# DinoBektesevic/lfd

Hardware: AMD Instinct MI355X
Metric: SDSS frames/sec (2048x1489) full detecttrails pipe (higher is better)
Workload: dtype f32

## Files before the change

lfd_amd/csrc/k_hough.h:

```cpp
#pragma once
#include "common.h"
#include "../../include/lfdmi.h"

#define PIXLIST_WORDS 8
#define CHUNK_MAX 64
__device__ __forceinline__ uint32_t chunk_entry(int y, int x0, int len) {
    return ((uint32_t)(len - 1) << 26) | ((uint32_t)y << 13) | (uint32_t)x0;
}

__global__ void __launch_bounds__(256)
k_pixlist(const u64 *bits0, const u64 *bits1, uint32_t *list0, uint32_t *list1, int *counters, int cm_a, int cm_b, int h, int w,
          size_t list_cap, int *accum_clear, int acc_n, size_t acc_stride, const int *active, int need_detect) {
    int g = blockIdx.y, im = blockIdx.z;
    const u64 *bits = im ? bits1 : bits0;
    uint32_t *list = im ? list1 : list0;
    const int cidx = im ? C_NPIX_BOX : C_NPIX_EQU, cidx_b = im ? C_NPIXB_BOX : C_NPIXB_EQU, nnz_idx = im ? C_NNZ_BOX : C_NNZ_EQU;
    if (accum_clear) accum_clear += (size_t)im * acc_stride;
    if (slot_off(active, counters, g)) return;
    int *cnt = counters + g * C_COUNT;
    if (need_detect && !cnt[C_DETECT]) return;
    int wq = LFD_WQ(w);
    if (accum_clear)
        for (int k = blockIdx.x * 256 + threadIdx.x; k < acc_n; k += gridDim.x * 256) accum_clear[(size_t)g * 2 * acc_stride + k] = 0;
    const int nw = h * wq;
// ... 199 lines not shown
    }
#undef LFD_BIN
    __syncthreads();
    int *ag = accum + ((size_t)g * 2 + im) * acc_cap;
    const int ts = numangle + 2;
    const int r0 = (numrho - 1) / 2 + lo;
    if (merge) {
        for (int k = threadIdx.x; k < nb * AW; k += NT) {
            int rr = r0 + (k >> aw_log2), al = k & (AW - 1);
            int v = acc[k];
            if (v && al < na) atomicAdd(&ag[(size_t)(rr + 1) * ts + a0 + al + 1], v);
        }
        return;
    }
    for (int k = threadIdx.x; k < (numrho + 2) * AW; k += NT) {
        int rr = (k >> aw_log2) - 1, al = k & (AW - 1);
        int rl = rr - r0;
        if (al < na) ag[(size_t)(rr + 1) * ts + a0 + al + 1] = (rl >= 0 && rl < nb) ? acc[rl * AW + al] : 0;
    }
    if (slab == 0)
        for (int k = threadIdx.x; k < numrho + 2; k += NT) { ag[(size_t)k * ts] = 0; ag[(size_t)k * ts + ts - 1] = 0; }
}

__global__ void __launch_bounds__(256)
k_hough_peaks(const int *accum, u64 *peaks, int *counters, int numangle, int numrho, int threshold,
              size_t acc_cap, size_t peak_cap, const int *active, int need_detect) {
    int g = blockIdx.z, im = blockIdx.y;
    if (slot_off(active, counters, g)) return;
    int *cnt = counters + g * C_COUNT;
    if (need_detect && !cnt[C_DETECT]) return;
    const int *ag = accum + ((size_t)g * 2 + im) * acc_cap;
    u64 *pg = peaks + ((size_t)g * 2 + im) * peak_cap;
    const int ts = numangle + 2;
    constexpr int PK_BUF = 4096;
    __shared__ u64 buf[PK_BUF];
    __shared__ int nbuf, gbase;
    if (threadIdx.x == 0) nbuf = 0;
    __syncthreads();
    auto flush = [&]() {
        const int nb = nbuf;
        if (threadIdx.x == 0 && nb) gbase = atomicAdd(&cnt[im ? C_NPEAK_BOX : C_NPEAK_EQU], nb);
        __syncthreads();
        for (int i = threadIdx.x; i < nb; i += (int)blockDim.x) {
            if ((size_t)(gbase + i) < peak_cap) pg[gbase + i] = buf[i];
            else cnt[C_OVERFLOW] = 1;
        }
        __syncthreads();
        if (threadIdx.x == 0) nbuf = 0;
        __syncthreads();
    };
    constexpr int RB = 8;
    const int per = ((numrho + (int)gridDim.x - 1) / (int)gridDim.x + RB - 1) / RB * RB;
    const int r0 = blockIdx.x * per, r1 = min(numrho, r0 + per);
    const int lane = threadIdx.x & 63, nth = (int)blockDim.x;
    int blk = 0;
    for (int n0 = 0; n0 < numangle; n0 += nth) {
        const int n = n0 + threadIdx.x;
        const bool on = n < numangle;
        const int *col = ag + (on ? n : 0) + 1;
        for (int rb = r0; rb < r1; rb += RB, blk++) {
            int v[RB + 2];
#pragma unroll
            for (int j = 0; j < RB + 2; j++) {
                const int rr = rb + j;
                v[j] = (on && rr <= numrho + 1) ? col[(size_t)rr * ts] : 0;
            }
#pragma unroll
            for (int j = 0; j < RB; j++) {
                const int r = rb + j, c = v[j + 1];
                int left = __shfl_up(c, 1), right = __shfl_down(c, 1);
                const bool cand = on && r < r1 && c > threshold && c > v[j] && c >= v[j + 2];
                if (cand) {
                    const int t = (r + 1) * ts + n + 1;
                    if (lane == 0) left = ag[t - 1];
                    if (lane == 63 || n == numangle - 1) right = ag[t + 1];
                    if (c > left && c >= right) {
                        const int base = (n + 1) * (numrho + 2) + r + 1;
                        buf[atomicAdd(&nbuf, 1)] = ((u64)(uint32_t)c << 32) | (u64)(uint32_t)(0x7fffffff - base);
                    }
                }
            }
            __syncthreads();
            if (nbuf > PK_BUF - RB * 256) flush();
            else __syncthreads();
        }
    }
    __syncthreads();
    flush();
}

__global__ void __launch_bounds__(256)
k_accum_untranspose(const int *accum, int *out, int numangle, int numrho, size_t acc_cap) {
    int g = blockIdx.y;
    const int *ag = accum + (size_t)g * 2 * acc_cap;
    int *og = out + (size_t)g * (numangle + 2) * (numrho + 2);
    int total = (numangle + 2) * (numrho + 2);
    for (int k = blockIdx.x * 256 + threadIdx.x; k < total; k += gridDim.x * 256) {
        int n1 = k / (numrho + 2), r1 = k - n1 * (numrho + 2);
        og[k] = ag[(size_t)r1 * (numangle + 2) + n1];
    }
}

__device__ __forceinline__ void key_to_line(u64 key, int numrho, float rho, float theta, float *orho,
                                            float *otheta) {
    int idx = 0x7fffffff - (int)(uint32_t)(key & 0xffffffffu);
    float scale = __fdiv_rn(1.f, (float)(numrho + 2));
    int n = (int)floorf(__fmul_rn((float)idx, scale)) - 1;
    int r = idx - (n + 1) * (numrho + 2) - 1;
    *orho = __fmul_rn(__fsub_rn((float)r, __fmul_rn((float)(numrho - 1), 0.5f)), rho);
    *otheta = __fadd_rn(0.f, __fmul_rn((float)n, theta));
}

__global__ void __launch_bounds__(256)
k_hough_topk(const u64 *peaks, const int *counters, float *lines, int K, int numrho, float rho,
             float theta, size_t peak_cap, const int *active, int need_detect) {
    int g = blockIdx.y, im = blockIdx.x;
    if (slot_off(active, counters, g)) return;
    const int *cnt = counters + g * C_COUNT;
    if (need_detect && !cnt[C_DETECT]) return;
    const u64 *pg = peaks + ((size_t)g * 2 + im) * peak_cap;
    int n = cnt[im ? C_NPEAK_BOX : C_NPEAK_EQU];
    if ((size_t)n > peak_cap) n = (int)peak_cap;
    __shared__ u64 red[4];
    __shared__ u64 prev_s;
    u64 prev = ~0ull;
    float *lg = lines + ((size_t)g * 2 + im) * K * 2;
    for (int round = 0; round < K; round++) {
        u64 best = 0;
        for (int k = threadIdx.x; k < n; k += 256) {
            u64 v = pg[k];
            if (v < prev && v > best) best = v;
        }
        for (int off = 32; off > 0; off >>= 1) {
            u64 o = __shfl_down(best, off);
            if (o > best) best = o;
        }
        if (lfd_lane() == 0) red[threadIdx.x >> 6] = best;
        __syncthreads();
        if (threadIdx.x == 0) {
            u64 b = red[0];
            for (int k = 1; k < 4; k++) if (red[k] > b) b = red[k];
            prev_s = b;
            float ro = 0.f, th = 0.f;
            if (b) key_to_line(b, numrho, rho, theta, &ro, &th);
            lg[2 * round] = ro;
            lg[2 * round + 1] = th;
        }
        __syncthreads();
        prev = prev_s;
        if (!prev) {
            if (threadIdx.x == 0)
                for (int r2 = round + 1; r2 < K; r2++) { lg[2 * r2] = 0.f; lg[2 * r2 + 1] = 0.f; }
            break;
        }
    }
}

__global__ void __launch_bounds__(1024)
k_hough_sort(u64 *peaks, const int *counters, float *lines, int max_lines, int numrho, float rho,
             float theta, size_t peak_cap) {
    int g = blockIdx.y, im = blockIdx.x;
    const int *cnt = counters + g * C_COUNT;
    if (cnt[C_OVERFLOW]) return;
    u64 *pg = peaks + ((size_t)g * 2 + im) * peak_cap;
    int n = cnt[im ? C_NPEAK_BOX : C_NPEAK_EQU];
    if ((size_t)n > peak_cap) n = (int)peak_cap;
    int np2 = 1;
    while (np2 < n) np2 <<= 1;
    for (int k = n + threadIdx.x; k < np2; k += 1024) pg[k] = 0;
    __syncthreads();
    for (int size = 2; size <= np2; size <<= 1)
        for (int stride = size >> 1; stride > 0; stride >>= 1) {
            for (int t = threadIdx.x; t < (np2 >> 1); t += 1024) {
                int lo = 2 * t - (t & (stride - 1));
                int hi = lo + stride;
                bool desc = ((lo & size) == 0);
                u64 a = pg[lo], b = pg[hi];
                if (desc ? (a < b) : (a > b)) { pg[lo] = b; pg[hi] = a; }
// ... 11 lines not shown
        for (int i = 0; i < n; i++) res = __dadd_rn(res, a[i]);
        return res;
    }
    double r[8], res;
    int i;
    for (int j = 0; j < 8; j++) r[j] = a[j];
    for (i = 8; i < n - (n % 8); i += 8)
        for (int j = 0; j < 8; j++) r[j] = __dadd_rn(r[j], a[i + j]);
    res = __dadd_rn(__dadd_rn(__dadd_rn(r[0], r[1]), __dadd_rn(r[2], r[3])),
                    __dadd_rn(__dadd_rn(r[4], r[5]), __dadd_rn(r[6], r[7])));
    for (; i < n; i++) res = __dadd_rn(res, a[i]);
    return res;
}
__device__ double np_mean_dev(const double *a, int n) {
    return __ddiv_rn(__dadd_rn(a[0], np_pairwise_dev(a + 1, n - 1)), (double)n);
}

struct TailParams {
    int navg;
    double dro, thetaTresh, lineSetTresh;
    int which;
};

__global__ void k_finalize(const float *lines, const int *counters, lfdmi_result *res, int *need_dim,
                           int *pass_flags, const int *active, TailParams tp, int G) {
    int g = blockIdx.x * blockDim.x + threadIdx.x;
    if (g >= G) return;
    if (active && !active[g]) { if (need_dim) need_dim[g] = 0; return; }
    const int *cnt = counters + g * C_COUNT;
    lfdmi_result r = res[g];
    r.detection = cnt[C_DETECT];
    r.rejected_by_theta = 0;
    r.n_lines_equ = r.n_lines_box = 0;
    if (cnt[C_OVERFLOW]) {
        r.status = LFDMI_ERR_CAPACITY;
        r.x1 = max(cnt[C_NRUNF], cnt[C_NRUNB]);
        r.y1 = cnt[C_NKEYS];
        r.x2 = cnt[C_NSLOTS];
        r.y2 = max(max(cnt[C_NPIX_EQU], cnt[C_NPIX_BOX]), max(cnt[C_NPIXB_EQU], cnt[C_NPIXB_BOX]));
        r.n_lines_equ = max(cnt[C_NPEAK_EQU], cnt[C_NPEAK_BOX]);
    }
    if (r.detection && r.status == 0) {
        int n1 = cnt[C_NPEAK_EQU], n2 = cnt[C_NPEAK_BOX];
        r.n_lines_equ = n1; r.n_lines_box = n2;
        if (n1 == 0 || n2 == 0) {
            r.status = LFDMI_ERR_NOLINES;
        } else {
            int K = tp.navg;
            const float *l1 = lines + ((size_t)g * 2 + 0) * K * 2, *l2 = lines + ((size_t)g * 2 + 1) * K * 2;
            double ro1[LFDMI_MAX_SET_LINES], ro2[LFDMI_MAX_SET_LINES], t1[LFDMI_MAX_SET_LINES],
                t2[LFDMI_MAX_SET_LINES];
            for (int i = 0; i < K; i++) {
                ro1[i] = ro2[i] = t1[i] = t2[i] = 0.;
                if (i >= n1) continue;
                ro1[i] = l1[2 * i];
                if (i >= n2) continue;
                ro2[i] = l2[2 * i];
                t1[i] = l1[2 * i + 1];
                t2[i] = l2[2 * i + 1];
            }
            bool rej = fabs(__dsub_rn(np_mean_dev(ro1, K), np_mean_dev(ro2, K))) > tp.dro;
            if (!rej) {
                double mx = t1[0], mn = t1[0];
                for (int i = 1; i < K; i++) { mx = fmax(mx, t1[i]); mn = fmin(mn, t1[i]); }
                rej = fabs(__dsub_rn(mx, mn)) > tp.thetaTresh;
            }
            if (!rej) {
                double mx = t2[0], mn = t2[0];
                for (int i = 1; i < K; i++) { mx = fmax(mx, t2[i]); mn = fmin(mn, t2[i]); }
                rej = fabs(__dsub_rn(mx, mn)) > tp.thetaTresh;
            }
            if (!rej) {
                for (int i = 0; i < K; i++) ro1[i] = fabs(__dsub_rn(t1[i], t2[i]));
                rej = np_mean_dev(ro1, K) > tp.lineSetTresh;
            }
            if (rej) r.rejected_by_theta = 1;
            else { r.found = tp.which; r.rho = l1[0]; r.theta = l1[1]; }
        }
    }
    res[g] = r;
    pass_flags[g] |= (tp.which == 1) ? (r.detection ? 1 : 0) : (2 | (r.detection ? 4 : 0));
    if (need_dim) need_dim[g] = (r.found == 0 && r.status == 0) ? 1 : 0;
}

__global__ void k_hough_reset(int *counters, int G) {
    int g = blockIdx.x * blockDim.x + threadIdx.x;
    if (g >= G) return;
    int *cnt = counters + g * C_COUNT;
    cnt[C_NPIX_EQU] = 0; cnt[C_NPIX_BOX] = 0; cnt[C_NPIXB_EQU] = 0; cnt[C_NPIXB_BOX] = 0; cnt[C_NPEAK_EQU] = 0; cnt[C_NPEAK_BOX] = 0;
    cnt[C_NNZ_EQU] = 0; cnt[C_NNZ_BOX] = 0;
}

__global__ void k_init_results(lfdmi_result *res, int *pass_flags, int G) {
    int g = blockIdx.x * blockDim.x + threadIdx.x;
    if (g >= G) return;
    pass_flags[g] = 0;
    lfdmi_result r;
    r.status = 0; r.found = 0; r.rho = 0.f; r.theta = 0.f;
    r.x1 = r.y1 = r.x2 = r.y2 = 0;
    r.n_lines_equ = r.n_lines_box = 0; r.detection = 0; r.rejected_by_theta = 0;
    res[g] = r;
}
```

lfd_amd/csrc/lfdmi.hip:

```cpp
#include <hip/hip_runtime.h>

#include <math.h>
#include <stdio.h>
#include <stdlib.h>
#include <time.h>
#include <pthread.h>
#include <sched.h>
#include <string.h>

#include <atomic>
#include <condition_variable>
#include <string>
#include <thread>
#include <mutex>
#include <memory>
#include <vector>

#include "../../include/lfdmi.h"
#include "common.h"
#include "k_ccl.h"
#include "k_hough.h"
#include "k_image.h"
#include "k_rect.h"
#include "k_frame.h"
#include "k_trail.h"
#include "fits_reader.h"
#include "unit.h"

#define LFD_PI 3.1415926535897932384626433832795
#define MAX_ANGLES 4096

enum {
    KID_REMOVESTARS = 0, KID_PREP_HIST, KID_LUT, KID_ERODE, KID_DILATE, KID_CANNY_NMS, KID_RUNS_INIT_FG,
    KID_RUNS_MERGE8, KID_RUNS_FLATTEN_FG, KID_EDGE, KID_RUNS_INIT_BG, KID_RUNS_MERGE4, KID_RUNS_FLATTEN_BG,
    KID_KEYS, KID_EXTREMES, KID_RECTS, KID_FILL, KID_PIXLIST, KID_VOTE, KID_PEAKS, KID_TOPK, KID_SORT,
    KID_FINALIZE, KID_DILATE_CANNY, KID_FRAME_FG, KID_FRAME_BG, KID_FRAME_KEYS, KID_PREP_ERODE, KID_PREP_DUAL, KID_BITS_ERODE, KID_MISC, TG_COUNT
};
static const char *const KID_NAMES[TG_COUNT] = {
    "k_removestars", "k_prep_hist", "k_lut", "k_morph(erode)", "k_morph(dilate)", "k_canny_nms", "k_runs_init(fg)",
    "k_runs_merge8", "k_runs_flatten(fg)", "k_edge_from_cand", "k_runs_init(bg)", "k_runs_merge4_bg",
    "k_runs_flatten(bg)", "k_keys", "k_extremes", "k_rects", "k_fill_quads", "k_pixlist", "k_hough_vote",
    "k_hough_peaks", "k_hough_topk", "k_hough_sort", "k_finalize", "k_dilate_canny", "k_frame_fg", "k_frame_bg",
    "k_frame_keys", "k_prep_erode", "k_prep_dual", "k_bits_erode", "misc"};

struct TimedSpan { hipEvent_t a, b; int group, pass, det; };

struct CallChunk {
    int c0, nc;
    bool general_on, scan_fused;
    long long growths;
};
struct PendingCall {
    int kind = 0;
// ... 70 lines not shown
    int *fb_fg = nullptr, *fb_bg = nullptr;
    int *perm = nullptr;
    const int *perm_cur = nullptr;
    bool use_perm = true;
    int *perm_tiles = nullptr;
    bool use_tile_perm = true;
    bool sky_fast = true;
    bool vote_classes = true;
    bool rs_fold_on = true;
    bool rs_fold = false;
    const int *rs_count_dev = nullptr; int rs_max_obj = 0;
    int rs_fill_at = 13;
    int rs_fill_at0 = 3, rs_fill_part = 0;
    float *rs_fill_frames = nullptr;
    int rs_fill_nc = 0, rs_fill_h = 0, rs_fill_w = 0;
    hipEvent_t ev_rsfill = nullptr;
    bool rs_fill_inflight = false;
    bool scan_fused = true;
    u64 *scan_partial = nullptr;
    int scan_epoch = 0;
    int scan_spin = 4096;
    bool rects_prep = true;
    bool vote_balance = true;
    lfdmi_result *res_dev = nullptr;
    void *res_host = nullptr;
    bool worst = false;
    lfdmi_ctx *spill = nullptr;
    long long n_spilled = 0;
    long long n_scan_giveups = 0, n_general_reruns = 0, n_general_chunks = 0, n_chunks = 0, n_cap_growths = 0;
    bool grow_on = true;
    bool scan_fused_cfg = true;
    int scan_quiet = 0, scan_rearm = 64;
    size_t bytes = 0;
    double min_rho = 1.0;
    void *scratch = nullptr;
    size_t scratch_bytes = 0;
    int last_h = 0, last_w = 0;
    int quiet_chunks = 0;
    void *feed_pin[2] = {nullptr, nullptr}, *feed_dev[2] = {nullptr, nullptr};
    size_t feed_bytes = 0, feed_pin_bytes = 0;
    bool feed_cpus_known = false;
    hipStream_t feed_copy = nullptr, feed_copy2 = nullptr;
    hipEvent_t feed_mid = nullptr;
    int feed_streams = 2;
    hipEvent_t feed_up[2] = {nullptr, nullptr};
    int feed_threads = 4;
// ... 245 lines not shown
    RET(dmalloc(ctx, &ctx->edgeb, G * BW));
    RET(dmalloc(ctx, &ctx->equb, G * BW));
    RET(dmalloc(ctx, &ctx->boxb, G * BW));
    RET(dmalloc(ctx, &ctx->dbits, G * BW));
    RET(dmalloc(ctx, &ctx->nzd, G * BW));
    for (int **p : {&ctx->Lf, &ctx->YMf, &ctx->FLf, &ctx->Lb, &ctx->YMb, &ctx->FLb, &ctx->SBf, &ctx->SBb, &ctx->PAb,
                    &ctx->ROWf, &ctx->ROWb})
        RET(dmalloc(ctx, p, G * ctx->run_cap));
    if (const char *e = getenv("LFDMI_DC_PROFILE")) ctx->dc_profile = atoi(e) != 0;
    if (const char *e = getenv("LFDMI_DC_SPECIALIZE")) ctx->dc_specialize = atoi(e) != 0;
    if (getenv("LFDMI_FRAME_PROFILE") || ctx->dc_profile) RET(dmalloc(ctx, &ctx->prof, G * 16));
    RET(dmalloc(ctx, &ctx->rsa, G * FRAME_RUNCAP));
    ctx->bm_bands = (max_h + CELLBM_ROWS - 1) / CELLBM_ROWS;
    if (const char *e = getenv("LFDMI_CELLBM")) ctx->use_cellbm = atoi(e) != 0;
    ctx->tile_cap = ((max_h + DCW_TH - 1) / DCW_TH) * ((max_w + CANNY_TW - 1) / CANNY_TW);
    RET(dmalloc(ctx, &ctx->tile_list, G * ctx->tile_cap));
    RET(dmalloc(ctx, &ctx->segcnt, G * SCAN_MAX_SEG));
    RET(dmalloc(ctx, &ctx->perm, G));
    RET(dmalloc(ctx, &ctx->perm_tiles, G));
    if (const char *e = getenv("LFDMI_TILE_PERM")) ctx->use_tile_perm = atoi(e) != 0;
    if (const char *e = getenv("LFDMI_SKY_FAST")) ctx->sky_fast = atoi(e) != 0;
    if (const char *e = getenv("LFDMI_VOTE_CLASSES")) ctx->vote_classes = atoi(e) != 0;
    if (const char *e = getenv("LFDMI_VOTE_BALANCE")) ctx->vote_balance = atoi(e) != 0;
    if (const char *e = getenv("LFDMI_RECTS_PREP")) ctx->rects_prep = atoi(e) != 0;
    if (const char *e = getenv("LFDMI_RS_FOLD")) ctx->rs_fold_on = atoi(e) != 0;
    if (const char *e = getenv("LFDMI_RS_SORT_MIN")) ctx->rs_sort_min = atoi(e);
    if (const char *e = getenv("LFDMI_SCAN_FUSED")) ctx->scan_fused = atoi(e) != 0;
    ctx->scan_fused_cfg = ctx->scan_fused;
    if (const char *e = getenv("LFDMI_GROW")) ctx->grow_on = atoi(e) != 0;
    if (const char *e = getenv("LFDMI_SCAN_REARM")) ctx->scan_rearm = std::max(1, atoi(e));
    if (const char *e = getenv("LFDMI_SCAN_SPIN")) ctx->scan_spin = std::max(0, atoi(e));
    if (const char *e = getenv("LFDMI_SCAN_EPOCH0")) ctx->scan_epoch = atoi(e) & ((1 << 22) - 1);
    if (const char *e = getenv("LFDMI_RS_FILL_AT")) ctx->rs_fill_at = atoi(e);
    if (const char *e = getenv("LFDMI_RS_FILL_AT0")) ctx->rs_fill_at0 = atoi(e);
    if (const char *e = getenv("LFDMI_PERM")) ctx->use_perm = atoi(e) != 0;
    RET(dmalloc(ctx, &ctx->fb_fg, G));
    RET(dmalloc(ctx, &ctx->fg_keys, G));
    HIPCHK(hipMemsetAsync(ctx->fg_keys, 0, G * sizeof(int), ctx->stream));
    if (const char *e = getenv("LFDMI_FG_KEYS")) ctx->fg_keys_on = atoi(e) != 0;
    RET(dmalloc(ctx, &ctx->fb_bg, G));
    RET(dmalloc(ctx, &ctx->scanf_, G * BW));
    RET(dmalloc(ctx, &ctx->scanb_, G * BW));
    RET(dmalloc(ctx, &ctx->keys, G * ctx->key_cap));
    RET(dmalloc(ctx, &ctx->bigkeys, G * ctx->key_cap));
    RET(dmalloc(ctx, &ctx->medkeys, G * ctx->key_cap));
    RET(dmalloc(ctx, &ctx->wl_fg, G * BW));
// ... 15 lines not shown
        ctx->counters = (int *)(blk + nb_bm + nb_hist);
        ctx->zero_block = blk;
        ctx->zero_bytes = nb_bm + nb_hist + nb_cnt;
        ctx->zero_counters_off = nb_bm + nb_hist;
        uint8_t *blk2 = nullptr;
        RET(dmalloc(ctx, &blk2, nb_bm + nb_hist));
        ctx->cellbm2 = (u64 *)blk2;
        ctx->hist2 = (int *)(blk2 + nb_bm);
        ctx->zero_block2 = blk2;
        ctx->zero_bytes2 = nb_bm + nb_hist;
        RET(dmalloc(ctx, &ctx->fullbits, G * (size_t)max_h * ((max_w + 255) >> 8)));
        RET(dmalloc(ctx, &ctx->candmask, G * (size_t)((max_h + MORPH_TH - 1) / MORPH_TH) * 2));
    }
    RET(dmalloc(ctx, &ctx->need_dim, G));
    RET(dmalloc(ctx, &ctx->scan_partial, G * SCAN_MAX_BLK));
    HIPCHK(hipMemsetAsync(ctx->scan_partial, 0, G * SCAN_MAX_BLK * sizeof(u64), ctx->stream));
    {
        char *blk = nullptr;
        RET(dmalloc(ctx, &blk, G * sizeof(int) + G * LFDMI_MAX_SCALES * sizeof(lfdmi_result)));
        ctx->pass_flags = (int *)blk;
        ctx->res_dev = (lfdmi_result *)(blk + G * sizeof(int));
        HIPCHK(hipHostMalloc(&ctx->res_host, G * sizeof(int) + G * sizeof(lfdmi_result), hipHostMallocDefault));
    }
    HIPCHK(hipFuncSetAttribute((const void *)k_hough_vote<6>, hipFuncAttributeMaxDynamicSharedMemorySize, 160 * 1024 - 64));
    HIPCHK(hipFuncSetAttribute((const void *)k_hough_vote<5>, hipFuncAttributeMaxDynamicSharedMemorySize, 160 * 1024 - 64));
    HIPCHK(hipFuncSetAttribute((const void *)k_hough_vote<4>, hipFuncAttributeMaxDynamicSharedMemorySize, 160 * 1024 - 64));
    HIPCHK(hipFuncSetAttribute((const void *)k_hough_vote<3>, hipFuncAttributeMaxDynamicSharedMemorySize, 160 * 1024 - 64));
    HIPCHK(hipFuncSetAttribute((const void *)k_hough_vote<2>, hipFuncAttributeMaxDynamicSharedMemorySize, 160 * 1024 - 64));
    HIPCHK(hipFuncSetAttribute((const void *)k_hough_vote<1>, hipFuncAttributeMaxDynamicSharedMemorySize, 160 * 1024 - 64));
    HIPCHK(hipFuncSetAttribute((const void *)k_hough_vote<0>, hipFuncAttributeMaxDynamicSharedMemorySize, 160 * 1024 - 64));
    HIPCHK(hipFuncSetAttribute((const void *)k_rects_big, hipFuncAttributeMaxDynamicSharedMemorySize, 160 * 1024 - 64));
    HIPCHK(hipFuncSetAttribute((const void *)k_dilate_canny_v, hipFuncAttributeMaxDynamicSharedMemorySize, 64 * 1024));
    HIPCHK(hipFuncSetAttribute((const void *)k_frame_fg, hipFuncAttributeMaxDynamicSharedMemorySize, 160 * 1024 - 1024));
    HIPCHK(hipFuncSetAttribute((const void *)k_prep_erode<false, 0>, hipFuncAttributeMaxDynamicSharedMemorySize, 140 * 1024));
    HIPCHK(hipFuncSetAttribute((const void *)k_prep_erode<false, 1>, hipFuncAttributeMaxDynamicSharedMemorySize, 140 * 1024));
    HIPCHK(hipFuncSetAttribute((const void *)k_prep_erode<false, 2>, hipFuncAttributeMaxDynamicSharedMemorySize, 140 * 1024));
    HIPCHK(hipFuncSetAttribute((const void *)k_prep_erode<false, 3>, hipFuncAttributeMaxDynamicSharedMemorySize, 140 * 1024));
    HIPCHK(hipFuncSetAttribute((const void *)k_prep_erode<true, LFDMI_PREP_BRIGHT_THEN_DIM>, hipFuncAttributeMaxDynamicSharedMemorySize, 140 * 1024));
    HIPCHK(hipFuncSetAttribute((const void *)k_frame_contours, hipFuncAttributeMaxDynamicSharedMemorySize,
                               (FRAME_RUNCAP + 4 * (FRAME_RUNCAP / 32)) * (int)sizeof(int)));
    HIPCHK(hipFuncSetAttribute((const void *)k_morph_rect<0>, hipFuncAttributeMaxDynamicSharedMemorySize, 64 * 1024));
    HIPCHK(hipFuncSetAttribute((const void *)k_morph_rect<1>, hipFuncAttributeMaxDynamicSharedMemorySize, 64 * 1024));
    return 0;
}

extern "C" int lfdmi_ctx_create(int device, int max_h, int max_w, int max_inflight, lfdmi_ctx **out) {
// ... 729 lines not shown
    float rho = (float)rho_d, theta = (float)theta_d;
    if (!(rho > 0) || !(theta > 0)) return fail(ctx, LFDMI_ERR_ARG, "rho and theta must be positive");
    int na, nr;
    lfdmi_hough_dims(h, w, rho_d, theta_d, &na, &nr);
    if (na <= 0 || nr <= 0 || na > MAX_ANGLES || (size_t)(na + 2) * (nr + 2) > ctx->acc_cap)
        return fail(ctx, LFDMI_ERR_CAPACITY, "Hough accumulator larger than the workspace (rho < 1 px or theta < 1 deg)");
    int slot = 0;
    for (int i = 1; i < LFDMI_MAX_SCALES; i++) if (ctx->tabs[i].stamp < ctx->tabs[slot].stamp) slot = i;
    auto &t = ctx->tabs[slot];
    t.host.assign((size_t)2 * na, 0.f);
    float irho = 1 / rho;
    float ang = 0.f;
    for (int n = 0; n < na; ang += theta, n++) {
        t.host[n] = (float)(cos((double)ang) * irho);
        t.host[na + n] = (float)(sin((double)ang) * irho);
    }
    HIPCHK(hipMemcpyAsync(ctx->tab + (size_t)slot * 2 * MAX_ANGLES, t.host.data(), t.host.size() * sizeof(float), hipMemcpyHostToDevice, ctx->stream));
    t.rho = rho_d; t.theta = theta_d; t.h = h; t.w = w; t.numangle = na; t.numrho = nr;
    t.stamp = ++ctx->tab_clock;
    ctx->tab_cur = slot; ctx->numangle = na; ctx->numrho = nr;
    return 0;
}

static int run_hough(lfdmi_ctx *ctx, int nc, int h, int w, double rho, double theta, int threshold, int n_img, int K,
                     int need_detect, const int *active) {
    RET(ensure_tables(ctx, h, w, rho, theta));
    int na = ctx->numangle, nr = ctx->numrho;
    const std::vector<float> &tab_host = ctx->tabs[ctx->tab_cur].host;
    const int half = (nr - 1) / 2;
    VoteRanges rng;
    int aw_log2 = 6, nslabs = 1, nbmax = nr;
    const bool have_tab = (int)tab_host.size() == 2 * na;
    auto slab_ranges = [&](int awl) {
        int AW = 1 << awl;
        nslabs = (na + AW - 1) / AW;
        nbmax = 1;
        for (int sl = 0; sl < VOTE_MAX_SLABS; sl++) { rng.lo[sl] = -half - 1; rng.hi[sl] = nr - half; }
        if (nslabs <= VOTE_MAX_SLABS && have_tab) {
            for (int sl = 0; sl < nslabs; sl++) {
                double rmin = 0, rmax = 0;
                for (int n = sl * AW; n < na && n < (sl + 1) * AW; n++) {
                    double c = tab_host[n], sn = tab_host[na + n];
                    for (int cx = 0; cx < 2; cx++)
                        for (int cy = 0; cy < 2; cy++) {
                            double r = (cx ? w : 0) * c + (cy ? h : 0) * sn;
                            rmin = r < rmin ? r : rmin;
                            rmax = r > rmax ? r : rmax;
                        }
// ... 61 lines not shown
                                                                    h, w, ctx->list_cap, (nsplit > 1 || balance) ? ctx->accum : nullptr, acc_n, ctx->acc_cap,
                                                                    active, need_detect);
        KCHK("k_pixlist"); }
        Span sp(ctx, KID_VOTE, need_detect);
        const int vsplit = balance ? 2 * nsplit : nsplit;
        dim3 vgrid(nslabs * vsplit, balance ? 1 : n_img, nc);
        size_t vlds = ((size_t)nbmax << aw_log2) * 4 + 256;
        static const int vote_threads_env = getenv("LFDMI_VOTE_THREADS") ? std::max(64, std::min(1024, atoi(getenv("LFDMI_VOTE_THREADS")) & ~63)) : 0;
        const int vote_threads = vote_threads_env ? vote_threads_env : (narrow_path ? VOTE_THREADS / 2 : VOTE_THREADS);
#define LFD_LAUNCH_VOTE(L)                                                                                          \
    case L:                                                                                                         \
        k_hough_vote<L><<<vgrid, vote_threads, vlds, ctx->stream>>>(ctx->pix_equ, ctx->pix_box, ctx->counters,           \
                                                                   ctx->tab + (size_t)ctx->tab_cur * 2 * MAX_ANGLES, \
                                                                   ctx->accum, na, nr, vsplit, ctx->list_cap,       \
                                                                   ctx->acc_cap, active, need_detect, rng, balance); \
        break;
        switch (aw_log2) {
            LFD_LAUNCH_VOTE(6) LFD_LAUNCH_VOTE(5) LFD_LAUNCH_VOTE(4) LFD_LAUNCH_VOTE(3) LFD_LAUNCH_VOTE(2)
            LFD_LAUNCH_VOTE(1) LFD_LAUNCH_VOTE(0)
        }
#undef LFD_LAUNCH_VOTE
        KCHK("k_hough_vote");
    }
    { Span sp(ctx, KID_PEAKS, need_detect);
    static const int peak_rows = getenv("LFDMI_PEAK_ROWS") ? std::max(8, atoi(getenv("LFDMI_PEAK_ROWS"))) : 32;
    k_hough_peaks<<<dim3(std::min(32, std::max(1, nr / peak_rows)), n_img, nc), std::min(256, (na + 63) / 64 * 64), 0, ctx->stream>>>(ctx->accum, ctx->peaks, ctx->counters, na, nr, threshold,
                                                                ctx->acc_cap, ctx->peak_cap, active, need_detect);
    KCHK("k_hough_peaks"); }
    if (K > 0) {
        Span sp(ctx, KID_TOPK, need_detect);
        k_hough_topk<<<dim3(n_img, nc), 256, 0, ctx->stream>>>(ctx->peaks, ctx->counters, ctx->lines, K, nr, (float)rho, (float)theta,
                                                               ctx->peak_cap, active, need_detect);
        KCHK("k_hough_topk");
    }
    return 0;
}

static int check_params(lfdmi_ctx *ctx, const lfdmi_params *p, bool dim) {
    if (!p) return fail(ctx, LFDMI_ERR_ARG, "params NULL");
    if (p->gaussKernel < 0 || p->gaussKernel > 31 || (p->gaussKernel > 0 && (p->gaussKernel & 1) == 0))
        return fail(ctx, LFDMI_ERR_ARG, "gaussKernel must be 0 (off) or odd, 1..31");
    if (p->nlinesInSet < 1 || p->nlinesInSet > LFDMI_MAX_SET_LINES) return fail(ctx, LFDMI_ERR_ARG, "nlinesInSet out of range");
    if (!p->dilateKernel) return fail(ctx, LFDMI_ERR_ARG, "dilateKernel NULL");
    if (dim && !p->erodeKernel) return fail(ctx, LFDMI_ERR_ARG, "erodeKernel NULL");
    return 0;
}

static int prep_erode_rows(const lfdmi_ctx *ctx, int w, int kh) {
    int BR = ctx->pe_rows;
// ... 117 lines not shown
    }
    if (p->gaussKernel > 0) {
        RET(run_morph(ctx, dil_src, ctx->equ, ctx->equb, ctx->lut, p->dilateKernel, p->dilate_kh, p->dilate_kw, 0, nc, h, w, active));
        RET(ensure_scratch(ctx, (size_t)ctx->G * ctx->N));
        RET(run_gauss(ctx, ctx->equ, (uint8_t *)ctx->scratch, nc, h, w, p->gaussKernel, p->gaussSigma, active));
        RET(run_canny(ctx, (const uint8_t *)ctx->scratch, nc, h, w, 0, 255, active, false, true));
    } else if (can_fuse_dilate_canny(p->dilateKernel, p->dilate_kh, p->dilate_kw, w)) {
        RET(run_dilate_canny(ctx, dil_src, nc, h, w, ctx->lut, p->dilate_kh, p->dilate_kw, active, ctx->use_cellbm ? bm : nullptr));
        RET(rs_fill_point(ctx, 2 + 10 * ctx->cur_pass));
        RET(run_canny(ctx, ctx->equ, nc, h, w, 0, 255, active, true, true));
    } else {
        RET(run_morph(ctx, dil_src, ctx->equ, ctx->equb, ctx->lut, p->dilateKernel, p->dilate_kh, p->dilate_kw, 0, nc, h, w, active));
        RET(run_canny(ctx, ctx->equ, nc, h, w, 0, 255, active, false, true));
    }
    return run_rects(ctx, nc, h, w, p->contoursMode, p->contoursMethod, p->minAreaRectMinLen, p->lwTresh, active);
}

static int run_tail(lfdmi_ctx *ctx, int nc, int h, int w, double rho, bool dim, const lfdmi_params *p, const int *active,
                    int *need_dim, lfdmi_result *res, bool again) {
    if (again) {
        k_hough_reset<<<(nc + 63) / 64, 64, 0, ctx->stream>>>(ctx->counters, nc);
        KCHK("k_hough_reset");
    }
    RET(run_hough(ctx, nc, h, w, rho, LFD_PI / 180, 1, 2, p->nlinesInSet, 1, active));
    TailParams tp;
    tp.navg = p->nlinesInSet; tp.dro = p->dro; tp.thetaTresh = p->thetaTresh; tp.lineSetTresh = p->lineSetTresh;
    tp.which = dim ? 2 : 1;
    Span sp(ctx, KID_FINALIZE);
    k_finalize<<<(nc + 63) / 64, 64, 0, ctx->stream>>>(ctx->lines, ctx->counters, res, need_dim, ctx->pass_flags, active, tp, nc);
    KCHK("k_finalize");
    return 0;
}

static int run_pass(lfdmi_ctx *ctx, const void *src, int dtype, int nc, int h, int w, int flip, int prep_mode, bool dim,
                    const lfdmi_params *p, const int *active, int *need_dim, const lfdmi_params *dual_dim = nullptr) {
    RET(run_front(ctx, src, dtype, nc, h, w, flip, prep_mode, dim, p, active, dual_dim));
    ctx->perm_cur = nullptr;
    return run_tail(ctx, nc, h, w, p->houghMethod, dim, p, active, need_dim, ctx->res_dev, false);
}

static void dictify(int h, int w, lfdmi_result *r) {
    if (!r->found) return;
    float c = cosf(r->theta), s = sinf(r->theta);
    float x0 = c * r->rho, y0 = s * r->rho;
    float L = (float)(h + w);
    r->x1 = (int32_t)(x0 - L * s);
    r->y1 = (int32_t)(y0 + L * c);
    r->x2 = (int32_t)(x0 + L * s);
    r->y2 = (int32_t)(y0 - L * c);
}
// ... 1271 lines not shown
    HIPCHK(hipSetDevice(ctx->device));
    const int G = ctx->G, K = navg;
    std::vector<float> lines((size_t)G * 2 * K * 2);
    std::vector<int> cnt((size_t)G * C_COUNT);
    for (int c0 = 0; c0 < n; c0 += G) {
        const int nc = std::min(G, n - c0);
        std::fill(lines.begin(), lines.end(), 0.f);
        std::fill(cnt.begin(), cnt.end(), 0);
        for (int i = 0; i < nc; i++) {
            const int a = n1[c0 + i], b = n2[c0 + i];
            if (a < 0 || a > kmax || b < 0 || b > kmax) return fail(ctx, LFDMI_ERR_ARG, "lfdmi_debug_tail: line count");
            for (int k = 0; k < K && k < a; k++) { lines[((size_t)i * 2 + 0) * K * 2 + 2 * k] = h1[((size_t)(c0 + i) * kmax + k) * 2]; lines[((size_t)i * 2 + 0) * K * 2 + 2 * k + 1] = h1[((size_t)(c0 + i) * kmax + k) * 2 + 1]; }
            for (int k = 0; k < K && k < b; k++) { lines[((size_t)i * 2 + 1) * K * 2 + 2 * k] = h2[((size_t)(c0 + i) * kmax + k) * 2]; lines[((size_t)i * 2 + 1) * K * 2 + 2 * k + 1] = h2[((size_t)(c0 + i) * kmax + k) * 2 + 1]; }
            cnt[(size_t)i * C_COUNT + C_DETECT] = 1;
            cnt[(size_t)i * C_COUNT + C_NPEAK_EQU] = a;
            cnt[(size_t)i * C_COUNT + C_NPEAK_BOX] = b;
        }
        HIPCHK(hipMemcpyAsync(ctx->lines, lines.data(), (size_t)nc * 2 * K * 2 * sizeof(float), hipMemcpyHostToDevice, ctx->stream));
        HIPCHK(hipMemcpyAsync(ctx->counters, cnt.data(), (size_t)nc * C_COUNT * sizeof(int), hipMemcpyHostToDevice, ctx->stream));
        k_init_results<<<(nc + 63) / 64, 64, 0, ctx->stream>>>(ctx->res_dev, ctx->pass_flags, nc);
        KCHK("k_init_results");
        TailParams tp;
        tp.navg = navg; tp.dro = dro; tp.thetaTresh = thetaTresh; tp.lineSetTresh = lineSetTresh; tp.which = which;
        k_finalize<<<(nc + 63) / 64, 64, 0, ctx->stream>>>(ctx->lines, ctx->counters, ctx->res_dev, nullptr, ctx->pass_flags, nullptr, tp, nc);
        KCHK("k_finalize");
        HIPCHK(hipMemcpyAsync(out + c0, ctx->res_dev, (size_t)nc * sizeof(lfdmi_result), hipMemcpyDeviceToHost, ctx->stream));
        HIPCHK(hipStreamSynchronize(ctx->stream));
        for (int i = 0; i < nc; i++) dictify(h, w, &out[c0 + i]);
    }
    return 0;
}

extern "C" int lfdmi_debug_trig(lfdmi_ctx *ctx, int n, const double *y, const double *x, float *angle_deg, float *cos_half, float *sin_half) {
    if (!ctx || n < 0 || !y || !x || !angle_deg || !cos_half || !sin_half) return LFDMI_ERR_ARG;
    RET(idle(ctx));
    if (n == 0) return 0;
    HIPCHK(hipSetDevice(ctx->device));
    RET(ensure_scratch(ctx, (size_t)n * (2 * sizeof(double) + 3 * sizeof(float))));
    double *dy = (double *)ctx->scratch, *dx = dy + n;
    float *o = (float *)(dx + n);
    HIPCHK(hipMemcpyAsync(dy, y, (size_t)n * sizeof(double), hipMemcpyHostToDevice, ctx->stream));
    HIPCHK(hipMemcpyAsync(dx, x, (size_t)n * sizeof(double), hipMemcpyHostToDevice, ctx->stream));
    k_debug_trig<<<(n + 255) / 256, 256, 0, ctx->stream>>>(dy, dx, o, o + n, o + 2 * (size_t)n, n);
    KCHK("k_debug_trig");
    HIPCHK(hipMemcpyAsync(angle_deg, o, (size_t)n * sizeof(float), hipMemcpyDeviceToHost, ctx->stream));
    HIPCHK(hipMemcpyAsync(cos_half, o + n, (size_t)n * sizeof(float), hipMemcpyDeviceToHost, ctx->stream));
    HIPCHK(hipMemcpyAsync(sin_half, o + 2 * (size_t)n, (size_t)n * sizeof(float), hipMemcpyDeviceToHost, ctx->stream));
    HIPCHK(hipStreamSynchronize(ctx->stream));
// ... 213 lines not shown
```

Baseline: 62780.

## Vectorize Hough peak scan and add optional fused peaks/topk/finalize tail kernel

```diff
diff --git a/lfd_amd/csrc/k_hough.h b/lfd_amd/csrc/k_hough.h
--- a/lfd_amd/csrc/k_hough.h
+++ b/lfd_amd/csrc/k_hough.h
@@ -245,6 +245,74 @@
         for (int k = threadIdx.x; k < numrho + 2; k += NT) { ag[(size_t)k * ts] = 0; ag[(size_t)k * ts + ts - 1] = 0; }
 }
 
+#define PEAK_ST 4
+__device__ __forceinline__ unsigned peak_item(const int *ag, int ts, int numangle, int r, int n0, int threshold, int *votes) {
+    const int *row = ag + (size_t)(r + 1) * ts + n0 + 1;
+    int c[PEAK_ST + 2], lo[PEAK_ST], hi[PEAK_ST];
+    if (n0 + PEAK_ST <= numangle) {
+        __builtin_memcpy(&c[1], row, PEAK_ST * sizeof(int));
+        __builtin_memcpy(lo, row - ts, PEAK_ST * sizeof(int));
+        __builtin_memcpy(hi, row + ts, PEAK_ST * sizeof(int));
+        c[0] = row[-1];
+        c[PEAK_ST + 1] = row[PEAK_ST];
+    } else {
+        c[0] = row[-1];
+#pragma unroll
+        for (int j = 0; j <= PEAK_ST; j++) c[j + 1] = (n0 + j <= numangle) ? row[j] : 0;
+#pragma unroll
+        for (int j = 0; j < PEAK_ST; j++) {
+            lo[j] = (n0 + j < numangle) ? row[j - ts] : 0;
+            hi[j] = (n0 + j < numangle) ? row[j + ts] : 0;
+        }
+    }
+    unsigned m = 0;
+#pragma unroll
+    for (int j = 0; j < PEAK_ST; j++) {
+        const int v = c[j + 1];
+        votes[j] = v;
+        if (n0 + j < numangle && v > threshold && v > lo[j] && v >= hi[j] && v > c[j] && v >= c[j + 2]) m |= 1u << j;
+    }
+    return m;
+}
+
+__device__ __forceinline__ void peaks_append(u64 *list, size_t cap, int *n, unsigned mask, const int *votes, int r, int n0, int numrho) {
+    const int lane = lfd_lane();
+    int off[PEAK_ST], total = 0;
+#pragma unroll
+    for (int j = 0; j < PEAK_ST; j++) {
+        const u64 bal = __ballot((mask >> j) & 1u);
+        off[j] = total + __popcll(bal & ((1ull << lane) - 1ull));
+        total += __popcll(bal);
+    }
+    if (total == 0) return;
+    int base = 0;
+    if (lane == 0) base = atomicAdd(n, total);
+    base = __shfl(base, 0);
+#pragma unroll
+    for (int j = 0; j < PEAK_ST; j++)
+        if ((mask >> j) & 1u) {
+            const int pos = base + off[j], cell = (n0 + j + 1) * (numrho + 2) + r + 1;
+            if ((size_t)pos < cap) list[pos] = ((u64)(uint32_t)votes[j] << 32) | (u64)(uint32_t)(0x7fffffff - cell);
+        }
+}
+
+__device__ __forceinline__ void peaks_scan(const int *ag, int numangle, int numrho, int threshold, int i_beg, int i_end, u64 *list,
+                                           size_t cap, int *n) {
+    const int ts = numangle + 2, nq = (numangle + PEAK_ST - 1) / PEAK_ST, nth = (int)blockDim.x;
+    for (int i0 = i_beg; i0 < i_end; i0 += nth) {
+        const int it = i0 + (int)threadIdx.x;
+        int votes[PEAK_ST] = {0, 0, 0, 0}, r = 0, n0 = 0;
+        unsigned m = 0;
+        if (it < i_end) {
+            const int dr = it / nq;
+            r = dr;
+            n0 = (it - dr * nq) * PEAK_ST;
+            m = peak_item(ag, ts, numangle, r, n0, threshold, votes);
+        }
+        peaks_append(list, cap, n, m, votes, r, n0, numrho);
+    }
+}
+
 __global__ void __launch_bounds__(256)
 k_hough_peaks(const int *accum, u64 *peaks, int *counters, int numangle, int numrho, int threshold,
               size_t acc_cap, size_t peak_cap, const int *active, int need_detect) {
@@ -254,8 +322,7 @@
     if (need_detect && !cnt[C_DETECT]) return;
     const int *ag = accum + ((size_t)g * 2 + im) * acc_cap;
     u64 *pg = peaks + ((size_t)g * 2 + im) * peak_cap;
-    const int ts = numangle + 2;
-    constexpr int PK_BUF = 4096;
+    constexpr int PK_BUF = 4096, PK_ROUND = 256 * PEAK_ST;
     __shared__ u64 buf[PK_BUF];
     __shared__ int nbuf, gbase;
     if (threadIdx.x == 0) nbuf = 0;
@@ -272,41 +339,14 @@
         if (threadIdx.x == 0) nbuf = 0;
         __syncthreads();
     };
-    constexpr int RB = 8;
-    const int per = ((numrho + (int)gridDim.x - 1) / (int)gridDim.x + RB - 1) / RB * RB;
-    const int r0 = blockIdx.x * per, r1 = min(numrho, r0 + per);
-    const int lane = threadIdx.x & 63, nth = (int)blockDim.x;
-    int blk = 0;
-    for (int n0 = 0; n0 < numangle; n0 += nth) {
-        const int n = n0 + threadIdx.x;
-        const bool on = n < numangle;
-        const int *col = ag + (on ? n : 0) + 1;
-        for (int rb = r0; rb < r1; rb += RB, blk++) {
-            int v[RB + 2];
-#pragma unroll
-            for (int j = 0; j < RB + 2; j++) {
-                const int rr = rb + j;
-                v[j] = (on && rr <= numrho + 1) ? col[(size_t)rr * ts] : 0;
-            }
-#pragma unroll
-            for (int j = 0; j < RB; j++) {
-                const int r = rb + j, c = v[j + 1];
-                int left = __shfl_up(c, 1), right = __shfl_down(c, 1);
-                const bool cand = on && r < r1 && c > threshold && c > v[j] && c >= v[j + 2];
-                if (cand) {
-                    const int t = (r + 1) * ts + n + 1;
-                    if (lane == 0) left = ag[t - 1];
-                    if (lane == 63 || n == numangle - 1) right = ag[t + 1];
-                    if (c > left && c >= right) {
-                        const int base = (n + 1) * (numrho + 2) + r + 1;
-                        buf[atomicAdd(&nbuf, 1)] = ((u64)(uint32_t)c << 32) | (u64)(uint32_t)(0x7fffffff - base);
-                    }
-                }
-            }
-            __syncthreads();
-            if (nbuf > PK_BUF - RB * 256) flush();
-            else __syncthreads();
-        }
+    const int per = (numrho + (int)gridDim.x - 1) / (int)gridDim.x;
+    const int r0 = min(numrho, (int)blockIdx.x * per), r1 = min(numrho, r0 + per);
+    const int nq = (numangle + PEAK_ST - 1) / PEAK_ST, i1 = r1 * nq;
+    for (int i0 = r0 * nq; i0 < i1; i0 += 256) {
+        peaks_scan(ag, numangle, numrho, threshold, i0, min(i1, i0 + 256), buf, PK_BUF, &nbuf);
+        __syncthreads();
+        if (nbuf > PK_BUF - PK_ROUND) flush();
+        else __syncthreads();
     }
     __syncthreads();
     flush();
@@ -332,6 +372,43 @@
     int r = idx - (n + 1) * (numrho + 2) - 1;
     *orho = __fmul_rn(__fsub_rn((float)r, __fmul_rn((float)(numrho - 1), 0.5f)), rho);
     *otheta = __fadd_rn(0.f, __fmul_rn((float)n, theta));
+}
+
+#define TOPK_MAX_WAVES 16
+__device__ __forceinline__ void topk_rounds(const u64 *pg, int n, float *lg, int K, int numrho, float rho, float theta,
+                                            u64 *red, u64 *prev_s_) {
+    u64 &prev_s = *prev_s_;
+    const int nth = (int)blockDim.x, nwv = nth >> 6;
+    u64 prev = ~0ull;
+    for (int round = 0; round < K; round++) {
+        u64 best = 0;
+        for (int k = threadIdx.x; k < n; k += nth) {
+            u64 v = pg[k];
+            if (v < prev && v > best) best = v;
+        }
+        for (int off = 32; off > 0; off >>= 1) {
+            u64 o = __shfl_down(best, off);
+            if (o > best) best = o;
+        }
+        if (lfd_lane() == 0) red[threadIdx.x >> 6] = best;
+        __syncthreads();
+        if (threadIdx.x == 0) {
+            u64 b = red[0];
+            for (int k = 1; k < nwv; k++) if (red[k] > b) b = red[k];
+            prev_s = b;
+            float ro = 0.f, th = 0.f;
+            if (b) key_to_line(b, numrho, rho, theta, &ro, &th);
+            lg[2 * round] = ro;
+            lg[2 * round + 1] = th;
+        }
+        __syncthreads();
+        prev = prev_s;
+        if (!prev) {
+            if (threadIdx.x == 0)
+                for (int r2 = round + 1; r2 < K; r2++) { lg[2 * r2] = 0.f; lg[2 * r2 + 1] = 0.f; }
+            break;
+        }
+    }
 }
 
 __global__ void __launch_bounds__(256)
@@ -344,39 +421,9 @@
     const u64 *pg = peaks + ((size_t)g * 2 + im) * peak_cap;
     int n = cnt[im ? C_NPEAK_BOX : C_NPEAK_EQU];
     if ((size_t)n > peak_cap) n = (int)peak_cap;
-    __shared__ u64 red[4];
+    __shared__ u64 red[TOPK_MAX_WAVES];
     __shared__ u64 prev_s;
-    u64 prev = ~0ull;
-    float *lg = lines + ((size_t)g * 2 + im) * K * 2;
-    for (int round = 0; round < K; round++) {
-        u64 best = 0;
-        for (int k = threadIdx.x; k < n; k += 256) {
-            u64 v = pg[k];
-            if (v < prev && v > best) best = v;
-        }
-        for (int off = 32; off > 0; off >>= 1) {
-            u64 o = __shfl_down(best, off);
-            if (o > best) best = o;
-        }
-        if (lfd_lane() == 0) red[threadIdx.x >> 6] = best;
-        __syncthreads();
-        if (threadIdx.x == 0) {
-            u64 b = red[0];
-            for (int k = 1; k < 4; k++) if (red[k] > b) b = red[k];
-            prev_s = b;
-            float ro = 0.f, th = 0.f;
-            if (b) key_to_line(b, numrho, rho, theta, &ro, &th);
-            lg[2 * round] = ro;
-            lg[2 * round + 1] = th;
-        }
-        __syncthreads();
-        prev = prev_s;
-        if (!prev) {
-            if (threadIdx.x == 0)
-                for (int r2 = round + 1; r2 < K; r2++) { lg[2 * r2] = 0.f; lg[2 * r2 + 1] = 0.f; }
-            break;
-        }
-    }
+    topk_rounds(pg, n, lines + ((size_t)g * 2 + im) * K * 2, K, numrho, rho, theta, red, &prev_s);
 }
 
 __global__ void __launch_bounds__(1024)
@@ -434,10 +481,8 @@
     int which;
 };
 
-__global__ void k_finalize(const float *lines, const int *counters, lfdmi_result *res, int *need_dim,
-                           int *pass_flags, const int *active, TailParams tp, int G) {
-    int g = blockIdx.x * blockDim.x + threadIdx.x;
-    if (g >= G) return;
+__device__ __forceinline__ void finalize_slot(int g, const float *lines, const int *counters, lfdmi_result *res, int *need_dim,
+                                              int *pass_flags, const int *active, const TailParams &tp, double *work) {
     if (active && !active[g]) { if (need_dim) need_dim[g] = 0; return; }
     const int *cnt = counters + g * C_COUNT;
     lfdmi_result r = res[g];
@@ -460,8 +505,7 @@
         } else {
             int K = tp.navg;
             const float *l1 = lines + ((size_t)g * 2 + 0) * K * 2, *l2 = lines + ((size_t)g * 2 + 1) * K * 2;
-            double ro1[LFDMI_MAX_SET_LINES], ro2[LFDMI_MAX_SET_LINES], t1[LFDMI_MAX_SET_LINES],
-                t2[LFDMI_MAX_SET_LINES];
+            double *ro1 = work, *ro2 = work + LFDMI_MAX_SET_LINES, *t1 = work + 2 * LFDMI_MAX_SET_LINES, *t2 = work + 3 * LFDMI_MAX_SET_LINES;
             for (int i = 0; i < K; i++) {
                 ro1[i] = ro2[i] = t1[i] = t2[i] = 0.;
                 if (i >= n1) continue;
@@ -493,6 +537,60 @@
     res[g] = r;
     pass_flags[g] |= (tp.which == 1) ? (r.detection ? 1 : 0) : (2 | (r.detection ? 4 : 0));
     if (need_dim) need_dim[g] = (r.found == 0 && r.status == 0) ? 1 : 0;
+}
+
+__global__ void k_finalize(const float *lines, const int *counters, lfdmi_result *res, int *need_dim,
+                           int *pass_flags, const int *active, TailParams tp, int G) {
+    int g = blockIdx.x * blockDim.x + threadIdx.x;
+    if (g >= G) return;
+    double work[4 * LFDMI_MAX_SET_LINES];
+    finalize_slot(g, lines, counters, res, need_dim, pass_flags, active, tp, work);
+}
+
+#define TAIL_THREADS 1024
+__global__ void __launch_bounds__(TAIL_THREADS)
+k_hough_tail(const int *accum, u64 *peaks, int *counters, float *lines, int numangle, int numrho, int threshold, int K,
+             float rho, float theta, size_t acc_cap, size_t peak_cap, int lds_cap, const int *active, int need_detect,
+             lfdmi_result *res, int *need_dim, int *pass_flags, TailParams tp) {
+    const int g = blockIdx.x;
+    extern __shared__ u64 lkeys[];
+    __shared__ u64 red[TOPK_MAX_WAVES];
+    __shared__ u64 prev_s;
+    __shared__ int nk;
+    __shared__ double work[4 * LFDMI_MAX_SET_LINES];
+    int *cnt = counters + g * C_COUNT;
+    if (accum && !slot_off(active, counters, g) && !(need_detect && !cnt[C_DETECT])) {
+        const int items = numrho * ((numangle + PEAK_ST - 1) / PEAK_ST);
+        bool ovf = false;
+        for (int im = 0; im < 2; im++) {
+            const int *ag = accum + ((size_t)g * 2 + im) * acc_cap;
+            u64 *pg = peaks + ((size_t)g * 2 + im) * peak_cap;
+            float *lg = lines + ((size_t)g * 2 + im) * K * 2;
+            if (threadIdx.x == 0) nk = 0;
+            __syncthreads();
+            peaks_scan(ag, numangle, numrho, threshold, 0, items, lkeys, (size_t)lds_cap, &nk);
+            __syncthreads();
+            const int n = nk;
+            if (n > lds_cap) {
+                __syncthreads();
+                if (threadIdx.x == 0) nk = 0;
+                __syncthreads();
+                peaks_scan(ag, numangle, numrho, threshold, 0, items, pg, peak_cap, &nk);
+                __syncthreads();
+                if ((size_t)n > peak_cap) {
+                    ovf = true;
+                    if (threadIdx.x == 0) cnt[C_OVERFLOW] = 1;
+                }
+            }
+            if (threadIdx.x == 0) cnt[im ? C_NPEAK_BOX : C_NPEAK_EQU] = n;
+            if (!ovf && K > 0) {
+                if (n > lds_cap) topk_rounds(pg, n, lg, K, numrho, rho, theta, red, &prev_s);
+                else topk_rounds(lkeys, n, lg, K, numrho, rho, theta, red, &prev_s);
+            }
+            __syncthreads();
+        }
+    }
+    if (res && threadIdx.x == 0) finalize_slot(g, lines, counters, res, need_dim, pass_flags, active, tp, work);
 }
 
 __global__ void k_hough_reset(int *counters, int G) {
diff --git a/lfd_amd/csrc/lfdmi.hip b/lfd_amd/csrc/lfdmi.hip
--- a/lfd_amd/csrc/lfdmi.hip
+++ b/lfd_amd/csrc/lfdmi.hip
@@ -29,6 +29,8 @@
 
 #define LFD_PI 3.1415926535897932384626433832795
 #define MAX_ANGLES 4096
+#define TAIL_LDS_KEYS_MAX 16384
+#define TAIL_FUSE_ITEMS 32768
 
 enum {
     KID_REMOVESTARS = 0, KID_PREP_HIST, KID_LUT, KID_ERODE, KID_DILATE, KID_CANNY_NMS, KID_RUNS_INIT_FG,
@@ -145,6 +147,8 @@
     int scan_spin = 4096;
     bool rects_prep = true;
     bool vote_balance = true;
+    bool fuse_tail = false;
+    int tail_lds_keys = 12288;
     lfdmi_result *res_dev = nullptr;
     void *res_host = nullptr;
     bool worst = false;
@@ -436,6 +440,8 @@
     if (const char *e = getenv("LFDMI_SKY_FAST")) ctx->sky_fast = atoi(e) != 0;
     if (const char *e = getenv("LFDMI_VOTE_CLASSES")) ctx->vote_classes = atoi(e) != 0;
     if (const char *e = getenv("LFDMI_VOTE_BALANCE")) ctx->vote_balance = atoi(e) != 0;
+    if (const char *e = getenv("LFDMI_FUSE_TAIL")) ctx->fuse_tail = atoi(e) != 0;
+    if (const char *e = getenv("LFDMI_TAIL_LDS_KEYS")) { int v = atoi(e); if (v >= 1 && v <= TAIL_LDS_KEYS_MAX) ctx->tail_lds_keys = v; }
     if (const char *e = getenv("LFDMI_RECTS_PREP")) ctx->rects_prep = atoi(e) != 0;
     if (const char *e = getenv("LFDMI_RS_FOLD")) ctx->rs_fold_on = atoi(e) != 0;
     if (const char *e = getenv("LFDMI_RS_SORT_MIN")) ctx->rs_sort_min = atoi(e);
@@ -497,6 +503,7 @@
         ctx->res_dev = (lfdmi_result *)(blk + G * sizeof(int));
         HIPCHK(hipHostMalloc(&ctx->res_host, G * sizeof(int) + G * sizeof(lfdmi_result), hipHostMallocDefault));
     }
+    HIPCHK(hipFuncSetAttribute((const void *)k_hough_tail, hipFuncAttributeMaxDynamicSharedMemorySize, TAIL_LDS_KEYS_MAX * (int)sizeof(u64)));
     HIPCHK(hipFuncSetAttribute((const void *)k_hough_vote<6>, hipFuncAttributeMaxDynamicSharedMemorySize, 160 * 1024 - 64));
     HIPCHK(hipFuncSetAttribute((const void *)k_hough_vote<5>, hipFuncAttributeMaxDynamicSharedMemorySize, 160 * 1024 - 64));
     HIPCHK(hipFuncSetAttribute((const void *)k_hough_vote<4>, hipFuncAttributeMaxDynamicSharedMemorySize, 160 * 1024 - 64));
@@ -1272,8 +1279,10 @@
     return 0;
 }
 
+struct TailFuse { TailParams tp; lfdmi_result *res; int *need_dim; bool done; };
+
 static int run_hough(lfdmi_ctx *ctx, int nc, int h, int w, double rho, double theta, int threshold, int n_img, int K,
-                     int need_detect, const int *active) {
+                     int need_detect, const int *active, TailFuse *fuse = nullptr) {
     RET(ensure_tables(ctx, h, w, rho, theta));
     int na = ctx->numangle, nr = ctx->numrho;
     const std::vector<float> &tab_host = ctx->tabs[ctx->tab_cur].host;
@@ -1381,9 +1390,20 @@
 #undef LFD_LAUNCH_VOTE
         KCHK("k_hough_vote");
     }
+    const long long tail_items = (long long)nr * ((na + PEAK_ST - 1) / PEAK_ST);
+    if (fuse && ctx->fuse_tail && n_img == 2 && K > 0 && tail_items <= TAIL_FUSE_ITEMS) {
+        const int lds_keys = (int)std::min<size_t>((size_t)ctx->tail_lds_keys, ctx->peak_cap);
+        Span sp(ctx, KID_PEAKS, need_detect);
+        k_hough_tail<<<nc, TAIL_THREADS, (size_t)lds_keys * sizeof(u64), ctx->stream>>>(
+            ctx->accum, ctx->peaks, ctx->counters, ctx->lines, na, nr, threshold, K, (float)rho, (float)theta, ctx->acc_cap, ctx->peak_cap,
+            lds_keys, active, need_detect, fuse->res, fuse->need_dim, ctx->pass_flags, fuse->tp);
+        KCHK("k_hough_tail");
+        fuse->done = true;
+        return 0;
+    }
     { Span sp(ctx, KID_PEAKS, need_detect);
     static const int peak_rows = getenv("LFDMI_PEAK_ROWS") ? std::max(8, atoi(getenv("LFDMI_PEAK_ROWS"))) : 32;
-    k_hough_peaks<<<dim3(std::min(32, std::max(1, nr / peak_rows)), n_img, nc), std::min(256, (na + 63) / 64 * 64), 0, ctx->stream>>>(ctx->accum, ctx->peaks, ctx->counters, na, nr, threshold,
+    k_hough_peaks<<<dim3(std::min(32, std::max(1, nr / peak_rows)), n_img, nc), 256, 0, ctx->stream>>>(ctx->accum, ctx->peaks, ctx->counters, na, nr, threshold,
                                                                 ctx->acc_cap, ctx->peak_cap, active, need_detect);
     KCHK("k_hough_peaks"); }
     if (K > 0) {
@@ -1547,10 +1567,13 @@
         k_hough_reset<<<(nc + 63) / 64, 64, 0, ctx->stream>>>(ctx->counters, nc);
         KCHK("k_hough_reset");
     }
-    RET(run_hough(ctx, nc, h, w, rho, LFD_PI / 180, 1, 2, p->nlinesInSet, 1, active));
-    TailParams tp;
+    TailFuse tf;
+    TailParams &tp = tf.tp;
     tp.navg = p->nlinesInSet; tp.dro = p->dro; tp.thetaTresh = p->thetaTresh; tp.lineSetTresh = p->lineSetTresh;
     tp.which = dim ? 2 : 1;
+    tf.res = res; tf.need_dim = need_dim; tf.done = false;
+    RET(run_hough(ctx, nc, h, w, rho, LFD_PI / 180, 1, 2, p->nlinesInSet, 1, active, &tf));
+    if (tf.done) return 0;
     Span sp(ctx, KID_FINALIZE);
     k_finalize<<<(nc + 63) / 64, 64, 0, ctx->stream>>>(ctx->lines, ctx->counters, res, need_dim, ctx->pass_flags, active, tp, nc);
     KCHK("k_finalize");
@@ -2868,8 +2891,15 @@
         KCHK("k_init_results");
         TailParams tp;
         tp.navg = navg; tp.dro = dro; tp.thetaTresh = thetaTresh; tp.lineSetTresh = lineSetTresh; tp.which = which;
+        if (ctx->fuse_tail) {
+            k_hough_tail<<<nc, TAIL_THREADS, (size_t)ctx->tail_lds_keys * sizeof(u64), ctx->stream>>>(
+                nullptr, ctx->peaks, ctx->counters, ctx->lines, 0, 0, 0, K, 0.f, 0.f, ctx->acc_cap, ctx->peak_cap, ctx->tail_lds_keys,
+                nullptr, 0, ctx->res_dev, nullptr, ctx->pass_flags, tp);
+            KCHK("k_hough_tail");
+        } else {
         k_finalize<<<(nc + 63) / 64, 64, 0, ctx->stream>>>(ctx->lines, ctx->counters, ctx->res_dev, nullptr, ctx->pass_flags, nullptr, tp, nc);
         KCHK("k_finalize");
+        }
         HIPCHK(hipMemcpyAsync(out + c0, ctx->res_dev, (size_t)nc * sizeof(lfdmi_result), hipMemcpyDeviceToHost, ctx->stream));
         HIPCHK(hipStreamSynchronize(ctx->stream));
         for (int i = 0; i < nc; i++) dictify(h, w, &out[c0 + i]);
```

Result: no change. 62730, median of 2 (-0.1%).
